# blacksnail789521/IMM-TSF

Hardware: AMD Instinct MI355X
Metric: forecast windows/sec (train fwd+bwd) on ragged 64-entity batch (higher is better)
Workload: dtype bf16

## Files before the change

imm-tsf_amd/csrc/gemm.hip:

```cpp
#include "gemm.hpp"
#include "rowops.hpp"
#include <atomic>
#include <mutex>
#include <shared_mutex>

namespace {

typedef short s16x4 __attribute__((ext_vector_type(4)));
typedef short s16x8 __attribute__((ext_vector_type(8)));

template <bool BF16> struct LdsElem { typedef float T; };
template <> struct LdsElem<true> { typedef bf16_t T; };

__device__ __forceinline__ float gelu_erf(float x) { return 0.5f * x * (1.f + erff(x * 0.70710678118654752f)); }
__device__ __forceinline__ float gelu_erf_grad(float z) {
    return 0.5f * (1.f + erff(z * 0.70710678118654752f)) + z * 0.3989422804014327f * expf(-0.5f * z * z);
}

template <bool BF16, bool TR, int ROWS, int BK> struct TileGeom {
    static constexpr bool kmajor = BF16 && TR;
    static constexpr int pad = BF16 ? 8 : 1;
    static constexpr int pitch = kmajor ? (ROWS + 8) : (BK + pad);
    static constexpr int elems = kmajor ? BK * pitch : ROWS * pitch;
};
// ... 593 lines not shown
    switch (layout) {
        case GEMM_NT: hipLaunchKernelGGL((gemm_kernel<BF16, false, false, BM, BN, BK, WM, WN, SPEC, BBF>), grid, block, 0, stream, g); break;
        case GEMM_NN: hipLaunchKernelGGL((gemm_kernel<BF16, false, true, BM, BN, BK, WM, WN, SPEC, BBF>), grid, block, 0, stream, g); break;
        case GEMM_TN:
            if (BBF) return IMMTSF_EINVAL;
            hipLaunchKernelGGL((gemm_kernel<BF16, true, true, BM, BN, BK, WM, WN, SPEC, false>), grid, block, 0, stream, g);
            break;
        default: return IMMTSF_EINVAL;
    }
    IMMTSF_LAUNCH_CHECK();
    return IMMTSF_OK;
}

static int g_force_old = 0;

int g_variant = 0, g_splitk = 0, g_xcd = 1, g_dbg = 0, g_tn_spec = 1, g_xcd2d = 0;

}

void immtsf_gemm_note_grid(long threads) { g_last_grid_threads = threads; }

extern int g_immtsf_ttcn_fused;
extern int g_immtsf_ttcn_bwd_grid;

extern "C" int immtsf_debug_gemm_config(int variant, int splitk) {
    g_immtsf_ttcn_fused = (variant & 0x8000) ? 0 : 1;
    g_variant = variant & 0xff;
    g_xcd = (variant & 0x100) ? 0 : 1;
    g_dbg = (variant >> 9) & 15;
    g_tn_spec = (variant & 0x2000) ? 0 : 1;
    g_xcd2d = (variant & 0x4000) ? 1 : 0;
    g_force_old = (variant & 0x10000) ? 1 : 0;
    g_immtsf_ttcn_bwd_grid = (variant >> 17) & 1023;
    g_splitk = splitk;
    return 0;
}

namespace {
struct TapRec { hipEvent_t e0, e1; int meta[10]; int members[24]; };
constexpr int kTapCap = 16384;
TapRec* g_tap = nullptr;
int g_tap_n = 0, g_tap_events = 0;
std::atomic<int> g_tap_on{0};
std::mutex g_tap_mu;
}

static int launch_gemm_impl(int layout, int precision, GemmArgs& g, hipStream_t stream);

namespace {
struct TwinRange { const float* base; const unsigned short* twin; size_t count; };
constexpr int kMaxTwins = 16;
TwinRange g_twins[kMaxTwins];
int g_ntwins = 0;
std::atomic<int> g_twins_on{1};
std::shared_mutex g_twins_mu;
}
// ... 375 lines not shown
```

imm-tsf_amd/csrc/ttcn.hip:

```cpp
#include "ttcn.hpp"
#include "../../include/immtsf.h"
#include "block_util.hpp"
#include "rowops.hpp"

int g_immtsf_ttcn_fused = 1;

namespace {

constexpr int LC = 32;

struct Dims { int P, L, F, K, NC, Fp, Kp, NCp, R; };
inline int r4(int x) { return (x + 31) / 32 * 32; }
inline Dims mk_dims(int P, int L, int te_dim, int K) {
    Dims d;
    d.P = P; d.L = L; d.F = 1 + te_dim; d.K = K; d.NC = d.F * K;
    d.Fp = r4(d.F); d.Kp = r4(K); d.NCp = r4(d.NC); d.R = P * L;
    return d;
}

__global__ __launch_bounds__(256) void build_x_kernel(Dims d, const float* __restrict__ x, const float* __restrict__ tt,
                                                       const float* ws, const float* bs, const float* __restrict__ wp,
                                                       const float* __restrict__ bp, float* __restrict__ X) {
    const long idx = (long)blockIdx.x * 256 + threadIdx.x;
    if (idx >= (long)d.R * d.Fp) return;
// ... 91 lines not shown
    const float* mp = mask + (size_t)p * d.L;
    for (int l0 = 0; l0 < d.L; l0 += LC) {
        const int lcnt = min(LC, d.L - l0);
        if (col) {
            for (int l = 0; l < lcnt; ++l) {
                const float smd = Sp[(size_t)(l0 + l) * d.NCp] * dpk;
                smt[l * d.NC + c] = smd;
                Sp[(size_t)(l0 + l) * d.NCp] = smd * (Xp[(size_t)(l0 + l) * d.Fp + fc] - ct) * mp[l0 + l];
            }
        }
        __syncthreads();
        for (int i = c; i < lcnt * d.Fp; i += nt) {
            const int l = i / d.Fp, f = i % d.Fp;
            float a = 0.f;
            if (f < d.F) for (int k = 0; k < d.K; ++k) a += smt[l * d.NC + k * d.F + f];
            dX[((size_t)p * d.L + l0 + l) * d.Fp + f] = a;
        }
        __syncthreads();
    }
}

struct Ws {
    float *X, *h1, *h2, *S, *ctr, *W1p, *b1p, *W2p, *b2p, *W3p, *b3p, *pack;
    size_t bytes;
};
Ws carve_ws(const Dims& d, void* base) {
    Carver k(base);
    Ws w;
    w.X = k.take<float>((size_t)d.R * d.Fp);
    w.h1 = k.take<float>((size_t)d.R * d.Kp);
    w.h2 = k.take<float>((size_t)d.R * d.Kp);
    w.S = k.take<float>((size_t)d.R * d.NCp);
    w.ctr = k.take<float>((size_t)d.P * (d.NC > d.F * 32 ? d.NC : d.F * 32));
    w.W1p = k.take<float>(d.Kp * d.Fp);
    w.b1p = k.take<float>(d.Kp);
    w.W2p = k.take<float>(d.Kp * d.Kp);
    w.b2p = k.take<float>(d.Kp);
    w.W3p = k.take<float>((size_t)d.NCp * d.Kp);
    w.b3p = k.take<float>(d.NCp);
    w.pack = k.take<float>(ttcn_full_pack_floats(d.F));
    w.bytes = k.bytes();
    return w;
}
struct Sc {
    float *dX, *dpool, *dz2, *dz1, *gW1p, *gb1p, *gW2p, *gb2p, *gW3p, *gb3p, *red, *slab;
    size_t bytes;
};
Sc carve_sc(const Dims& d, void* base) {
    Carver k(base);
    Sc s;
    s.dX = k.take<float>((size_t)d.R * d.Fp);
    s.dpool = k.take<float>((size_t)d.P * d.K);
    s.dz2 = k.take<float>((size_t)d.R * d.Kp);
    s.dz1 = k.take<float>((size_t)d.R * d.Kp);
    s.gW1p = k.take<float>(d.Kp * d.Fp);
    s.gb1p = k.take<float>(d.Kp);
    s.gW2p = k.take<float>(d.Kp * d.Kp);
    s.gb2p = k.take<float>(d.Kp);
    s.gW3p = k.take<float>((size_t)d.NCp * d.Kp);
    s.gb3p = k.take<float>(d.NCp);
    s.red = k.take<float>(64 * (d.NCp + 64) + 2 * 256 * d.F);
    s.slab = k.take<float>(ttcn_full_slab_floats(d.F));
    s.bytes = k.bytes();
// ... 33 lines not shown
int immtsf_patch_flatten3(const float* x, const float* tt, const float* mask, int32_t B, int32_t M, int32_t L, int32_t N, float* ox,
                          float* ott, float* omask, immtsf_stream_t stream) {
    if (!x || !tt || !mask || !ox || !ott || !omask || B < 0 || M <= 0 || L <= 0 || N <= 0) return IMMTSF_EINVAL;
    const size_t total = (size_t)B * M * L * N;
    if (total == 0) return IMMTSF_OK;
    hipLaunchKernelGGL(patch_flatten3_kernel, dim3((unsigned)((total + 255) / 256)), dim3(256), 0, static_cast<hipStream_t>(stream), x, tt, mask,
                       B, M, L, N, ox, ott, omask);
    IMMTSF_LAUNCH_CHECK();
    return IMMTSF_OK;
}

int immtsf_ttcn_forward(int32_t P, int32_t L, int32_t te_dim, int32_t ttcn_dim, int32_t precision, const float* x,
                        const float* tt, const float* mask, const immtsf_ttcn_params* p, float* out, int32_t out_ld,
                        int32_t flag_col, void* workspace, size_t workspace_bytes, immtsf_stream_t stream) {
    if (!x || !tt || !mask || !p || !out || !workspace) return IMMTSF_EINVAL;
    if (out_ld < ttcn_dim || flag_col >= out_ld || (flag_col >= 0 && flag_col < ttcn_dim)) return IMMTSF_EINVAL;
    if (bad_dims(P, L, te_dim, ttcn_dim)) return (1 + te_dim) * ttcn_dim > 1024 ? IMMTSF_EUNSUPPORTED : IMMTSF_EINVAL;
    if (P == 0) return IMMTSF_OK;
    const Dims d = mk_dims(P, L, te_dim, ttcn_dim);
    Ws w = carve_ws(d, workspace);
    if (workspace_bytes < w.bytes) return IMMTSF_EWORKSPACE;
    hipStream_t s = static_cast<hipStream_t>(stream);
    if (g_immtsf_ttcn_fused && ttcn_full_supported(precision, L, d.F, d.K))
        return launch_ttcn_full_fwd(P, L, d.F, d.K, x, tt, mask, p, w.pack, w.ctr, out, out_ld, flag_col, s);
    PackPtrs q{p->W1, p->b1, p->W2, p->b2, p->W3, p->b3, w.W1p, w.b1p, w.W2p, w.b2p, w.W3p, w.b3p};
    hipLaunchKernelGGL(pack_w_kernel, dim3(cdiv(d.NCp * d.Kp, 256)), dim3(256), 0, s, d, q);
    IMMTSF_LAUNCH_CHECK();
    const long nx = (long)d.R * d.Fp;
    hipLaunchKernelGGL(build_x_kernel, dim3((unsigned)((nx + 255) / 256)), dim3(256), 0, s, d, x, tt, p->te_scale_w, p->te_scale_b,
                       p->te_per_w, p->te_per_b, w.X);
    IMMTSF_LAUNCH_CHECK();
    {
        GemmArgs g = gemm_args(d.R, d.Kp, d.Fp, d.Fp, d.Fp, d.Kp);
        set_problem(g, 0, w.X, w.W1p, w.h1, w.b1p);
        g.act = 1;
        CHECK(immtsf_launch_gemm(GEMM_NT, precision, g, s));
    }
    {
        GemmArgs g = gemm_args(d.R, d.Kp, d.Kp, d.Kp, d.Kp, d.Kp);
        set_problem(g, 0, w.h1, w.W2p, w.h2, w.b2p);
        g.act = 1;
        CHECK(immtsf_launch_gemm(GEMM_NT, precision, g, s));
    }
    {
        GemmArgs g = gemm_args(d.R, d.NCp, d.Kp, d.Kp, d.Kp, d.NCp);
        set_problem(g, 0, w.h2, w.W3p, w.S, w.b3p);
        CHECK(immtsf_launch_gemm(GEMM_NT, precision, g, s));
    }
    const int threads = cdiv(d.NC, 64) * 64;
    hipLaunchKernelGGL(pool_fwd_kernel, dim3(P), dim3(threads), d.NC * sizeof(float), s, d, w.S, w.X, mask, p->T_bias, w.ctr, out, out_ld, flag_col);
    IMMTSF_LAUNCH_CHECK();
    return IMMTSF_OK;
}

int immtsf_ttcn_backward(int32_t P, int32_t L, int32_t te_dim, int32_t ttcn_dim, int32_t precision, const float* x,
                         const float* tt, const float* mask, const immtsf_ttcn_params* p, const float* out,
                         const float* dout, int32_t out_ld, void* workspace, size_t workspace_bytes, void* scratch,
                         size_t scratch_bytes, const immtsf_ttcn_params* gr, int32_t te_accumulate, immtsf_stream_t stream) {
    if (!tt || !mask || !p || !out || !dout || !gr || !workspace || !scratch || out_ld < ttcn_dim) return IMMTSF_EINVAL;
    if (bad_dims(P, L, te_dim, ttcn_dim)) return IMMTSF_EINVAL;
    if (P == 0) return IMMTSF_OK;
    const Dims d = mk_dims(P, L, te_dim, ttcn_dim);
    Ws w = carve_ws(d, workspace);
    Sc sc = carve_sc(d, scratch);
    if (workspace_bytes < w.bytes || scratch_bytes < sc.bytes) return IMMTSF_EWORKSPACE;
    hipStream_t s = static_cast<hipStream_t>(stream);
    if (g_immtsf_ttcn_fused && ttcn_full_supported(precision, L, d.F, d.K))
        return launch_ttcn_full_bwd(P, L, d.F, d.K, x, tt, mask, p, w.pack, w.ctr, out, dout, out_ld, sc.slab, gr,
                                    static_cast<hipStream_t>(stream), te_accumulate);
    {
        const size_t nbytes = (size_t)((char*)(sc.gb3p + d.NCp) - (char*)sc.gW1p);
        if (int rc = launch_fill(sc.gW1p, 0.f, nbytes / sizeof(float), s)) return rc;
    }
    Fork fk(s);
    {
        const int threads = cdiv(d.NC, 64) * 64;
        const size_t lds = (size_t)(d.K + LC * d.NC) * sizeof(float);
        if (lds > 160 * 1024) return IMMTSF_EUNSUPPORTED;
        hipLaunchKernelGGL(pool_bwd_kernel, dim3(P), dim3(threads), lds, s, d, w.S, w.X, mask, w.ctr, out, dout, out_ld, sc.dX, sc.dpool);
        IMMTSF_LAUNCH_CHECK();
    }
    CHECK(launch_colsum(sc.dpool, nullptr, P, nullptr, d.K, d.K, gr->T_bias, 0, sc.red, s));
    {
        GemmArgs h = gemm_args(d.NCp, d.Kp, d.R, d.NCp, d.Kp, d.Kp);
        set_problem(h, 0, w.S, w.h2, sc.gW3p, nullptr, sc.gb3p);
        h.c_prezeroed = 1;
        CHECK(immtsf_launch_gemm(GEMM_TN, precision, h, fk.fork()));
        GemmArgs g = gemm_args(d.R, d.Kp, d.NCp, d.NCp, d.Kp, d.Kp);
        set_problem(g, 0, w.S, w.W3p, sc.dz2, nullptr);
        g.relu_ref = w.h2; g.ld_ref = d.Kp;
        CHECK(immtsf_launch_gemm(GEMM_NN, precision, g, s));
// ... 31 lines not shown
```

imm-tsf_amd/csrc/ttcn.hpp:

```cpp
#pragma once
#include "common.hpp"

struct immtsf_ttcn_params;
bool ttcn_full_supported(int precision, int L, int F, int K);
size_t ttcn_full_pack_floats(int F);
size_t ttcn_full_slab_floats(int F);
int launch_ttcn_full_fwd(int P, int L, int F, int K, const float* x, const float* tt, const float* mask, const immtsf_ttcn_params* p,
                         float* pack, float* ctr, float* out, int out_ld, int flag_col, hipStream_t s);
int launch_ttcn_full_bwd(int P, int L, int F, int K, const float* x, const float* tt, const float* mask, const immtsf_ttcn_params* p,
                         const float* pack, const float* ctr, const float* out, const float* dout, int out_ld, float* slab,
                         const immtsf_ttcn_params* gr, hipStream_t s, int te_acc = 0);
```

imm-tsf_amd/csrc/ttcn_full.hip:

```cpp
#include "ttcn.hpp"
#include "../../include/immtsf.h"
#include "common.hpp"
#include <stdio.h>
#include <stdlib.h>

int g_immtsf_ttcn_bwd_grid = 0;

namespace {

typedef short s16x8 __attribute__((ext_vector_type(8)));
typedef float f32x2 __attribute__((ext_vector_type(2)));

constexpr int KP = 32;
constexpr int PT = 40;


struct FD { int P, L, F, K, NCq, dbg; };

struct Slab { int W1, b1, W2, b2, W3, b3, te, Tb, total; };
__host__ __device__ inline Slab slab_of(int F) {
    Slab s;
    int o = 0;
    s.W1 = o; o += KP * KP;
    s.b1 = o; o += KP;
    s.W2 = o; o += KP * KP;
    s.b2 = o; o += KP;
    s.W3 = o; o += F * 32 * KP;
    s.b3 = o; o += F * 32;
    s.te = o; o += 2 * KP;
    s.Tb = o; o += KP;
    s.total = o;
    return s;
}

__device__ __forceinline__ bf16x8 load8_bf16(const float* __restrict__ src) {
    const float4 a = *reinterpret_cast<const float4*>(src), b = *reinterpret_cast<const float4*>(src + 4);
    bf16x8 r;
// ... 102 lines not shown
        const f32x4 acc = mfma(frag_row(in, PT, rt * 16, 0, fr, fq), load8_bf16(W + (nt * 16 + fr) * KP + fq * 8), zero4());
        const float bias = b[nt * 16 + fr];
#pragma unroll
        for (int r = 0; r < 4; ++r) outp[(rt * 16 + fq * 4 + r) * PT + nt * 16 + fr] = (bf16_t)fmaxf(acc[r] + bias, 0.f);
    }
}

template <int RT>
__device__ __forceinline__ void mlp_layer_frag(const bf16_t* in, bf16_t* outp, const bf16x8 wf, const float bias, int wave, int fr, int fq) {
    for (int t = wave; t < RT * 2; t += 4) {
        const int rt = t >> 1, nt = t & 1;
        const f32x4 acc = mfma(frag_row(in, PT, rt * 16, 0, fr, fq), wf, zero4());
#pragma unroll
        for (int r = 0; r < 4; ++r) outp[(rt * 16 + fq * 4 + r) * PT + nt * 16 + fr] = (bf16_t)fmaxf(acc[r] + bias, 0.f);
    }
}

struct Wts { const float *W1p, *b1p, *W2p, *b2p, *W3q, *b3q; };

template <int RT, int MF>
__global__ __launch_bounds__(256) void ttcn_full_fwd_kernel(FD d, const float* __restrict__ x, const float* __restrict__ tt,
                                                             const float* __restrict__ mask, TEp te, Wts w, const bf16_t* __restrict__ W3h,
                                                             const float* __restrict__ Tb, float* __restrict__ ctr,
                                                             float* __restrict__ out, int out_ld, int flag_col) {
    extern __shared__ __attribute__((aligned(16))) unsigned char smem[];
    constexpr int ROWS = RT * 16, XP = xt_pitch<RT>();
    constexpr float LOG2E = 1.4426950408889634f;
    bf16_t* Xb = reinterpret_cast<bf16_t*>(smem);
    bf16_t* h1s = Xb + ROWS * PT;
    bf16_t* h2s = h1s + ROWS * PT;
    float* Xf = reinterpret_cast<float*>(h2s + ROWS * PT);
    float* cl = Xf + 16 * XP;
    float* pin = cl + d.NCq;
    const int tid = threadIdx.x, lane = tid & 63, wave = tid >> 6, fr = lane & 15, fq = lane >> 4;
    bf16x8 bw[MF][2];
    float b3v[MF][2];
    const int tnt = wave & 1;
    typedef PatchIn<RT, false> PI;
    PI nx;
    nx.fetch(d, blockIdx.x, x, tt, mask, nullptr, nullptr, nullptr, 0);
    const XCol xc = x_col(d, te);
    const bf16x8 mw1 = load8_bf16(w.W1p + (tnt * 16 + fr) * KP + fq * 8), mw2 = load8_bf16(w.W2p + (tnt * 16 + fr) * KP + fq * 8);
    const float mb1 = w.b1p[tnt * 16 + fr], mb2 = w.b2p[tnt * 16 + fr];
    const float tb = tid < d.K ? Tb[tid] : 0.f;
#pragma unroll
    for (int j = 0; j < MF; ++j)
#pragma unroll
        for (int half = 0; half < 2; ++half) {
            const int f = wave + 4 * j, c = f * 32 + half * 16 + fr;
            bw[j][half] = bf16x8{0, 0, 0, 0, 0, 0, 0, 0};
            b3v[j][half] = 0.f;
            if (f < d.F) { bw[j][half] = *reinterpret_cast<const bf16x8*>(W3h + (size_t)c * KP + fq * 8); b3v[j][half] = w.b3q[c] * LOG2E; }
        }
    nx.park(d, pin);
    __syncthreads();
    int it = 0;
    for (int p = blockIdx.x; p < d.P; p += gridDim.x, ++it) {
    const float* cur = pin + (it & 1) * PI::HEAD;
    const int pn = p + gridDim.x;
    if (pn < d.P) nx.fetch(d, pn, x, tt, mask, nullptr, nullptr, nullptr, 0);
    build_x<RT, true>(d, xc, cur, Xb, Xf);
    __syncthreads();
    mlp_layer_frag<RT>(Xb, h1s, mw1, mb1, wave, fr, fq);
    __syncthreads();
    mlp_layer_frag<RT>(h1s, h2s, mw2, mb2, wave, fr, fq);
    __syncthreads();
    bf16x8 a[RT];
    bool on[RT][4];
    float cval[RT][4];
#pragma unroll
    for (int rt = 0; rt < RT; ++rt) {
        a[rt] = frag_row(h2s, PT, rt * 16, 0, fr, fq);
        const f32x4 m4 = *reinterpret_cast<const f32x4*>(cur + 2 * ROWS + rt * 16 + fq * 4);
#pragma unroll
        for (int r = 0; r < 4; ++r) {
            on[rt][r] = m4[r] != 0.f;
            cval[rt][r] = rt * 16 + fq * 4 + r < d.L ? -1e8f * LOG2E : -INFINITY;
        }
    }
#pragma unroll
    for (int j = 0; j < MF; ++j) {
        const int f = wave + 4 * j;
        if (f < d.F) {
// ... 23 lines not shown
                            m = fmaxf(m, v[rt][h][e]);
                        }
                }
                m = col_max(m);
                f32x2 s2{0.f, 0.f}, p2{0.f, 0.f};
#pragma unroll
                for (int rt = 0; rt < RT; ++rt)
#pragma unroll
                    for (int h = 0; h < 2; ++h) {
                        v[rt][h] -= m;
                        v[rt][h][0] = __builtin_amdgcn_exp2f(v[rt][h][0]);
                        v[rt][h][1] = __builtin_amdgcn_exp2f(v[rt][h][1]);
                        s2 += v[rt][h];
                        p2 += v[rt][h] * xf[rt][h];
                    }
                const float acc = col_sum(p2[0] + p2[1]) * __builtin_amdgcn_rcpf(col_sum(s2[0] + s2[1]));
                if (fq == 0) {
                    cl[c] = acc;
                    ctr[(size_t)p * d.NCq + c] = acc;
                }
            }
        }
    }
    if (pn < d.P) nx.park(d, pin + ((it + 1) & 1) * PI::HEAD);
    __syncthreads();
    if (tid < d.K) {
        float s = tb;
        for (int f = 0; f < d.F; ++f) s += cl[f * 32 + tid];
        out[(size_t)p * out_ld + tid] = fmaxf(s, 0.f);
    }
    if (flag_col >= 0 && wave == 1) {
        float any = lane < d.L ? cur[2 * ROWS + lane] : 0.f;
        any = wave_sum(any);
        if (lane == 0) out[(size_t)p * out_ld + flag_col] = any > 0.f ? 1.f : 0.f;
    }
    __syncthreads();
    }
}

struct WtsT { const bf16_t *W3T , *W2T , *W1T , *W3h ; };

template <int RT, int MF>
__global__ __launch_bounds__(256) __attribute__((amdgpu_waves_per_eu(RT == 2 ? 2 : 1))) void ttcn_full_bwd_kernel(FD d, const float* __restrict__ x, const float* __restrict__ tt,
                                                             const float* __restrict__ mask, TEp te, Wts w, WtsT wt,
                                                             const float* __restrict__ ctr, const float* __restrict__ out,
                                                             const float* __restrict__ dout, int out_ld, float* __restrict__ slab) {
    extern __shared__ __attribute__((aligned(16))) unsigned char smem[];
    constexpr int ROWS = RT * 16, PTT = ROWS + 8, XP = xt_pitch<RT>();
    constexpr float LOG2E = 1.4426950408889634f;
    bf16_t* Xb = reinterpret_cast<bf16_t*>(smem);
    bf16_t* h1s = Xb + ROWS * PT;
    bf16_t* h2s = h1s + ROWS * PT;
    bf16_t* dz2s = h2s + ROWS * PT;
    bf16_t* dz1s = h2s;
    bf16_t* dST = dz2s + ROWS * PT;
    float* Xf = reinterpret_cast<float*>(dST + d.NCq * PTT);
    float* Xc = Xf + 16 * XP;
    typedef PatchIn<RT, true> PI;
    const int PIN = PI::HEAD + d.NCq;
    float* pin = Xc + 16 * XP;
    bf16_t* W3s = reinterpret_cast<bf16_t*>(pin + 2 * PIN);
    bf16_t* W1s = W3s + d.NCq * PT;
    bf16_t* W2s = W1s + KP * PT;
    float* b3s = reinterpret_cast<float*>(W2s + KP * PT);
    const int tid = threadIdx.x, lane = tid & 63, wave = tid >> 6, fr = lane & 15, fq = lane >> 4;
    const Slab sl = slab_of(d.F);
    PI nx;
    nx.fetch(d, blockIdx.x, x, tt, mask, ctr, out, dout, out_ld);
    const XCol xc = x_col(d, te);
    for (int i = tid; i < d.NCq * 4; i += 256) {
        const int c = i >> 2, q = i & 3;
        *reinterpret_cast<bf16x8*>(W3s + c * PT + q * 8) = *reinterpret_cast<const bf16x8*>(wt.W3h + (size_t)c * KP + q * 8);
    }
    for (int i = tid; i < d.NCq; i += 256) b3s[i] = w.b3q[i] * LOG2E;
    if (tid < 2 * KP * 4) {
        const int which = tid >> 7, r = (tid >> 2) & 31, q = tid & 3;
        *reinterpret_cast<bf16x8*>((which ? W2s : W1s) + r * PT + q * 8) = load8_bf16((which ? w.W2p : w.W1p) + r * KP + q * 8);
    }

    f32x4 accW3[MF][2][2];
    f32x2 accB3[MF][2];
#pragma unroll
    for (int j = 0; j < MF; ++j)
#pragma unroll
        for (int half = 0; half < 2; ++half) {
            accW3[j][half][0] = zero4(); accW3[j][half][1] = zero4();
            accB3[j][half] = f32x2{0.f, 0.f};
        }
    const int tnt = wave & 1, tmt = wave >> 1;
    const float mb1 = w.b1p[tnt * 16 + fr], mb2 = w.b2p[tnt * 16 + fr];
    f32x4 accW2 = zero4(), accW1 = zero4();
    float sb2 = 0.f, sb1 = 0.f;
    float accT = 0.f;
    float te_w = 0.f, te_b = 0.f;
    f32x2 tpw[MF], tpb[MF];
#pragma unroll
    for (int j = 0; j < MF; ++j) tpw[j] = tpb[j] = f32x2{0.f, 0.f};

    nx.park(d, pin);
    __syncthreads();
    int it = 0;
    for (int p = blockIdx.x; p < d.P; p += gridDim.x, ++it) {
        const float* cur = pin + (it & 1) * PIN;
        const float *dp = cur + 3 * ROWS, *cts = cur + PI::HEAD;
        const int pn = p + gridDim.x;
        if (pn < d.P) nx.fetch(d, pn, x, tt, mask, ctr, out, dout, out_ld);
        build_x<RT, true>(d, xc, cur, Xb, Xf, Xc);
        __syncthreads();
        if (tid >= 128 && tid < 128 + KP) accT += dp[tid - 128];
        mlp_layer_frag<RT>(Xb, h1s, frag_row(W1s, PT, tnt * 16, 0, fr, fq), mb1, wave, fr, fq);
        __syncthreads();
        mlp_layer_frag<RT>(h1s, h2s, frag_row(W2s, PT, tnt * 16, 0, fr, fq), mb2, wave, fr, fq);
        __syncthreads();
        bf16x8 a[RT];
        bool on[RT][4];
        float cval[RT][4], anyf = 0.f;
        f32x4 t4[RT];
#pragma unroll
        for (int rt = 0; rt < RT; ++rt) {
            a[rt] = frag_row(h2s, PT, rt * 16, 0, fr, fq);
            t4[rt] = *reinterpret_cast<const f32x4*>(cur + rt * 16 + fq * 4);
            const f32x4 m4 = *reinterpret_cast<const f32x4*>(cur + 2 * ROWS + rt * 16 + fq * 4);
#pragma unroll
            for (int r = 0; r < 4; ++r) {
                on[rt][r] = m4[r] != 0.f;
                cval[rt][r] = rt * 16 + fq * 4 + r < d.L ? -1e8f * LOG2E : -INFINITY;
                anyf += on[rt][r] ? 1.f : 0.f;
            }
        }
// ... 108 lines not shown
                const int o = (rt * 16 + fq * 4 + r) * PT + tnt * 16 + fr;
                const float g = (float)h1s[o] > 0.f ? acc[r] : 0.f;
                dz1s[o] = (bf16_t)g;
                sb1 += g;
            }
        }
        __syncthreads();
        if (wave < 2) {
#pragma unroll
            for (int kk = 0; kk < ROWS; kk += 32)
                accW1 = mfma(frag_kmajor(dz1s, PT, wave * 16, kk, fr, fq), frag_kmajor(Xb, PT, 0, kk, fr, fq), accW1);
        }
        for (int rt = (RT == 2 ? wave - 2 : wave); rt >= 0 && rt < RT; rt += 4) {
            const f32x4 acc = mfma(frag_row(dz1s, PT, rt * 16, 0, fr, fq), frag_kmajor(W1s, PT, 0, 0, fr, fq), zero4());
            const f32x4 c4 = *reinterpret_cast<const f32x4*>(Xc + fr * XP + rt * 16 + fq * 4);
            const f32x4 tr = *reinterpret_cast<const f32x4*>(cur + rt * 16 + fq * 4);
#pragma unroll
            for (int r = 0; r < 4; ++r) {
                const float g = acc[r] * c4[r];
                te_w = fmaf(g, tr[r], te_w);
                te_b += g;
            }
        }
        if (pn < d.P) nx.park(d, pin + ((it + 1) & 1) * PIN);
        __syncthreads();
    }

    float* my = slab + (size_t)blockIdx.x * sl.total;
#pragma unroll
    for (int j = 0; j < MF; ++j) {
        const int f = wave + 4 * j;
        if (f < d.F) {
#pragma unroll
            for (int half = 0; half < 2; ++half) {
#pragma unroll
                for (int nt = 0; nt < 2; ++nt)
#pragma unroll
                    for (int r = 0; r < 4; ++r)
                        my[sl.W3 + (size_t)(f * 32 + half * 16 + fq * 4 + r) * KP + nt * 16 + fr] = accW3[j][half][nt][r];
                const float b3sum = col_sum(accB3[j][half][0] + accB3[j][half][1]);
                if (fq == 0) my[sl.b3 + f * 32 + half * 16 + fr] = b3sum;
            }
        }
    }
#pragma unroll
    for (int r = 0; r < 4; ++r) {
        my[sl.W2 + (tmt * 16 + fq * 4 + r) * KP + tnt * 16 + fr] = accW2[r];
        if (wave < 2) my[sl.W1 + (wave * 16 + fq * 4 + r) * KP + fr] = accW1[r];
    }
    if (tid >= 128 && tid < 128 + KP) my[sl.Tb + tid - 128] = accT;
    float* tes = pin;
    if (tid < 4 * KP) tes[tid] = 0.f;
    __syncthreads();
#pragma unroll
    for (int j = 0; j < MF; ++j) {
        const int f = wave + 4 * j;
        const float sw = col_sum(row_sum16(tpw[j][0] + tpw[j][1])), sb = col_sum(row_sum16(tpb[j][0] + tpb[j][1]));
        if (lane == 0 && f >= 1 && f < d.F) {
            atomicAdd(tes + f, sw);
            atomicAdd(tes + KP + f, sb);
        }
    }
    te_w = col_sum(te_w);
    te_b = col_sum(te_b);
    sb2 = col_sum(sb2);
    sb1 = col_sum(sb1);
    if (fq == 0) {
        if (RT == 4 || wave >= 2) {
            atomicAdd(tes + fr, te_w);
            atomicAdd(tes + KP + fr, te_b);
        }
        atomicAdd(tes + 2 * KP + tnt * 16 + fr, sb2);
        atomicAdd(tes + 3 * KP + tnt * 16 + fr, sb1);
    }
    __syncthreads();
    if (tid < 2 * KP) my[sl.te + tid] = tes[tid];
    else if (tid < 3 * KP) my[sl.b2 + tid - 2 * KP] = tes[tid];
    else if (tid < 4 * KP) my[sl.b1 + tid - 3 * KP] = tes[tid];
}

struct PackIn { const float *W1, *b1, *W2, *b2, *W3, *b3; };
__global__ __launch_bounds__(256) void ttcn_pack_kernel(int F, int K, PackIn q, float* W1p, float* b1p, float* W2p, float* b2p,
                                                         float* W3q, float* b3q, bf16_t* W3T, bf16_t* W2T, bf16_t* W1T, bf16_t* W3h) {
    const int i = blockIdx.x * 256 + threadIdx.x, NCq = F * 32;
    if (i < KP * KP) {
        const int r = i >> 5, c = i & 31;
        const float v1 = (r < K && c < F) ? q.W1[r * F + c] : 0.f, v2 = (r < K && c < K) ? q.W2[r * K + c] : 0.f;
        W1p[i] = v1;
        W2p[i] = v2;
        W1T[c * KP + r] = (bf16_t)v1;
        W2T[c * KP + r] = (bf16_t)v2;
    }
    if (i < KP) { b1p[i] = i < K ? q.b1[i] : 0.f; b2p[i] = i < K ? q.b2[i] : 0.f; }
    if (i < NCq * KP) {
        const int c = i >> 5, kk = i & 31, f = c >> 5, k = c & 31;
        const float v = (k < K && kk < K) ? q.W3[(size_t)(k * F + f) * K + kk] : 0.f;
        W3q[i] = v;
        W3T[(size_t)kk * NCq + c] = (bf16_t)v;
        W3h[i] = (bf16_t)v;
    }
    if (i < NCq) { const int f = i >> 5, k = i & 31; b3q[i] = k < K ? q.b3[k * F + f] : 0.f; }
}

struct UnpackOut { float *W1, *b1, *W2, *b2, *W3, *b3, *ws, *bs, *wp, *bp, *Tb; };
__global__ __launch_bounds__(256) void ttcn_unpack_kernel(int F, int K, const float* __restrict__ slab, int nslab, UnpackOut g, int te_acc) {
    __shared__ float red[8][33];
    const Slab sl = slab_of(F);
    const int slot = threadIdx.x & 31, part = threadIdx.x >> 5;
    int i = blockIdx.x * 32 + slot, n;
    float* dst = nullptr;
    int off = 0;
    bool acc = false;
    if (i < (n = K * F)) { dst = g.W1 + i; off = sl.W1 + (i / F) * KP + i % F; }
    else if ((i -= n) < (n = K * K)) { dst = g.W2 + i; off = sl.W2 + (i / K) * KP + i % K; }
    else if ((i -= n) < (n = F * K * K)) { const int c = i / K, kk = i % K, k = c / F, f = c % F; dst = g.W3 + i; off = sl.W3 + (f * 32 + k) * KP + kk; }
    else if ((i -= n) < (n = F * K)) { const int k = i / F, f = i % F; dst = g.b3 + i; off = sl.b3 + f * 32 + k; }
    else if ((i -= n) < K) { dst = g.b1 + i; off = sl.b1 + i; }
    else if ((i -= K) < K) { dst = g.b2 + i; off = sl.b2 + i; }
    else if ((i -= K) < K) { dst = g.Tb + i; off = sl.Tb + i; }
    else if ((i -= K) < 1) { dst = g.ws; off = sl.te + 1; acc = te_acc != 0; }
    else if ((i -= 1) < 1) { dst = g.bs; off = sl.te + KP + 1; acc = te_acc != 0; }
    else if ((i -= 1) < F - 2) { dst = g.wp + i; off = sl.te + 2 + i; acc = te_acc != 0; }
    else if ((i -= F - 2) < F - 2) { dst = g.bp + i; off = sl.te + KP + 2 + i; acc = te_acc != 0; }
    float s = 0.f;
    if (dst) {
#pragma unroll 8
        for (int w = part; w < nslab; w += 8) s += slab[(size_t)w * sl.total + off];
    }
    red[part][slot] = s;
    __syncthreads();
    if (part == 0 && dst) {
#pragma unroll
        for (int q = 1; q < 8; ++q) s += red[q][slot];
        *dst = (acc ? *dst : 0.f) + s;
    }
}
inline int ttcn_unpack_outputs(int F, int K) { return K * F + K * K + F * K * K + F * K + 3 * K + 2 + 2 * (F - 2); }
constexpr int kMaxBwdGrid = 512;

size_t fwd_lds(int RT, int NCq) { return (size_t)RT * 16 * PT * 2 * 3 + (size_t)16 * (RT * 16 + 4) * 4 + (size_t)NCq * 4 + (size_t)2 * 3 * RT * 16 * 4 + 64; }
size_t bwd_lds(int RT, int NCq) {
    const size_t ROWS = RT * 16;
    return ROWS * PT * 2 * 4 + (size_t)NCq * (ROWS + 8) * 2 + 16 * (ROWS + 4) * 4 * 2 + 2 * (3 * ROWS + KP + (size_t)NCq) * 4 + (size_t)(NCq + 2 * KP) * PT * 2 + (size_t)NCq * 4;
}

struct PackPtrs { float *W1p, *b1p, *W2p, *b2p, *W3q, *b3q; bf16_t *W3T, *W2T, *W1T, *W3h; };
PackPtrs pack_ptrs(float* base, int F) {
    PackPtrs q;
    float* o = base;
    q.W1p = o; o += KP * KP;
    q.W2p = o; o += KP * KP;
    q.b1p = o; o += KP;
    q.b2p = o; o += KP;
    q.W3q = o; o += (size_t)F * 32 * KP;
    q.b3q = o; o += F * 32;
    q.W3T = reinterpret_cast<bf16_t*>(o); o += (size_t)F * 32 * KP / 2;
    q.W2T = reinterpret_cast<bf16_t*>(o); o += KP * KP / 2;
    q.W1T = reinterpret_cast<bf16_t*>(o); o += KP * KP / 2;
    q.W3h = reinterpret_cast<bf16_t*>(o);
    return q;
}

}

bool ttcn_full_supported(int precision, int L, int F, int K) {
    return precision == 1 && K >= 1 && K <= 32 && F >= 2 && F <= 16 && L >= 1 && L <= 64;
}
size_t ttcn_full_pack_floats(int F) { return (size_t)2 * KP * KP + 2 * KP + (size_t)F * 32 * KP + F * 32 + (size_t)F * 32 * KP + KP * KP + 64; }
size_t ttcn_full_slab_floats(int F) { return (size_t)kMaxBwdGrid * slab_of(F).total; }

int launch_ttcn_full_fwd(int P, int L, int F, int K, const float* x, const float* tt, const float* mask, const immtsf_ttcn_params* p,
                         float* pack, float* ctr, float* out, int out_ld, int flag_col, hipStream_t s) {
    const FD d{P, L, F, K, F * 32};
    const PackPtrs q = pack_ptrs(pack, F);
    hipLaunchKernelGGL(ttcn_pack_kernel, dim3(cdiv(F * 32 * KP, 256)), dim3(256), 0, s, F, K, PackIn{p->W1, p->b1, p->W2, p->b2, p->W3, p->b3},
                       q.W1p, q.b1p, q.W2p, q.b2p, q.W3q, q.b3q, q.W3T, q.W2T, q.W1T, q.W3h);
    IMMTSF_LAUNCH_CHECK();
    const TEp te{p->te_scale_w, p->te_scale_b, p->te_per_w, p->te_per_b};
    const Wts w{q.W1p, q.b1p, q.W2p, q.b2p, q.W3q, q.b3q};
    const int mf = (F + 3) / 4;
#define TTCN_FWD(RT, MF)                                                                                                                     \
    hipLaunchKernelGGL((ttcn_full_fwd_kernel<RT, MF>), dim3(P < 2048 ? P : 2048), dim3(256), fwd_lds(RT, d.NCq), s, d, x, tt, mask, te, w, q.W3h, p->T_bias, ctr, \
                       out, out_ld, flag_col)
    if (L <= 32) {
        if (mf == 1) TTCN_FWD(2, 1); else if (mf == 2) TTCN_FWD(2, 2); else if (mf == 3) TTCN_FWD(2, 3); else TTCN_FWD(2, 4);
    } else {
        if (mf == 1) TTCN_FWD(4, 1); else if (mf == 2) TTCN_FWD(4, 2); else if (mf == 3) TTCN_FWD(4, 3); else TTCN_FWD(4, 4);
    }
#undef TTCN_FWD
    IMMTSF_LAUNCH_CHECK();
    return IMMTSF_OK;
}

int launch_ttcn_full_bwd(int P, int L, int F, int K, const float* x, const float* tt, const float* mask, const immtsf_ttcn_params* p,
                         const float* pack, const float* ctr, const float* out, const float* dout, int out_ld, float* slab,
                         const immtsf_ttcn_params* gr, hipStream_t s, int te_acc) {
    const FD d{P, L, F, K, F * 32, 0};
    const PackPtrs q = pack_ptrs(const_cast<float*>(pack), F);
    const TEp te{p->te_scale_w, p->te_scale_b, p->te_per_w, p->te_per_b};
    const Wts w{q.W1p, q.b1p, q.W2p, q.b2p, q.W3q, q.b3q};
    const WtsT wt{q.W3T, q.W2T, q.W1T, q.W3h};
    const int genv = g_immtsf_ttcn_bwd_grid;
    int gmax = genv > 0 ? genv : (L <= 32 ? (P >= 8192 ? 512 : 384) : 224);
    gmax = gmax > kMaxBwdGrid ? kMaxBwdGrid : gmax;
    const int grid = P < gmax ? P : gmax;
    const size_t lds = bwd_lds(L <= 32 ? 2 : 4, d.NCq);
    const int mf = (F + 3) / 4;
#define TTCN_BWD(RT, MF)                                                                                                                  \
    do {                                                                                                                                  \
        if (lds > 64 * 1024)                                                                                                              \
            (void)hipFuncSetAttribute(reinterpret_cast<const void*>(ttcn_full_bwd_kernel<RT, MF>), hipFuncAttributeMaxDynamicSharedMemorySize, \
                                      (int)lds);                                                                                          \
        hipLaunchKernelGGL((ttcn_full_bwd_kernel<RT, MF>), dim3(grid), dim3(256), lds, s, d, x, tt, mask, te, w, wt, ctr, out, dout, out_ld, \
                           slab);                                                                                                         \
    } while (0)
    if (L <= 32) {
        if (mf == 1) TTCN_BWD(2, 1); else if (mf == 2) TTCN_BWD(2, 2); else if (mf == 3) TTCN_BWD(2, 3); else TTCN_BWD(2, 4);
    } else {
        if (mf == 1) TTCN_BWD(4, 1); else if (mf == 2) TTCN_BWD(4, 2); else if (mf == 3) TTCN_BWD(4, 3); else TTCN_BWD(4, 4);
    }
#undef TTCN_BWD
    IMMTSF_LAUNCH_CHECK();
    hipLaunchKernelGGL(ttcn_unpack_kernel, dim3(cdiv(ttcn_unpack_outputs(F, K), 32)), dim3(256), 0, s, F, K, slab, grid,
                       UnpackOut{gr->W1, gr->b1, gr->W2, gr->b2, gr->W3, gr->b3, gr->te_scale_w, gr->te_scale_b, gr->te_per_w, gr->te_per_b,
                                 gr->T_bias}, te_acc);
    IMMTSF_LAUNCH_CHECK();
    return IMMTSF_OK;
}
```

Before: 156,700.

## Skip MLP for fully-masked TTCN patches and rebalance backward work lists

The forward kernel detects patches whose mask is entirely zero, records a per-patch live flag, and takes a short path that computes only the masked-mean centre instead of running the full MLP. The backward kernel builds per-block work lists from those flags, spreading live and dead patches evenly across blocks. Dead patches get a cheap gradient path that touches only the time-embedding and T_bias terms. Blocks left without work can exit early, and the unpack kernel reads how many slabs were actually written. This targets the wasted work on ragged batches with many empty patches, at the cost of extra LDS, a prefix scan, and more code complexity.

```diff
diff --git a/imm-tsf_amd/csrc/gemm.hip b/imm-tsf_amd/csrc/gemm.hip
--- a/imm-tsf_amd/csrc/gemm.hip
+++ b/imm-tsf_amd/csrc/gemm.hip
@@ -639,6 +639,7 @@
 
 extern int g_immtsf_ttcn_fused;
 extern int g_immtsf_ttcn_bwd_grid;
+extern int g_immtsf_ttcn_live;
 
 extern "C" int immtsf_debug_gemm_config(int variant, int splitk) {
     g_immtsf_ttcn_fused = (variant & 0x8000) ? 0 : 1;
@@ -649,6 +650,7 @@
     g_xcd2d = (variant & 0x4000) ? 1 : 0;
     g_force_old = (variant & 0x10000) ? 1 : 0;
     g_immtsf_ttcn_bwd_grid = (variant >> 17) & 1023;
+    g_immtsf_ttcn_live = 7 & ~(variant >> 27);
     g_splitk = splitk;
     return 0;
 }
diff --git a/imm-tsf_amd/csrc/ttcn.hip b/imm-tsf_amd/csrc/ttcn.hip
--- a/imm-tsf_amd/csrc/ttcn.hip
+++ b/imm-tsf_amd/csrc/ttcn.hip
@@ -137,6 +137,7 @@
 
 struct Ws {
     float *X, *h1, *h2, *S, *ctr, *W1p, *b1p, *W2p, *b2p, *W3p, *b3p, *pack;
+    unsigned char* live;
     size_t bytes;
 };
 Ws carve_ws(const Dims& d, void* base) {
@@ -154,6 +155,7 @@
     w.W3p = k.take<float>((size_t)d.NCp * d.Kp);
     w.b3p = k.take<float>(d.NCp);
     w.pack = k.take<float>(ttcn_full_pack_floats(d.F));
+    w.live = k.take<unsigned char>(ttcn_full_live_bytes());
     w.bytes = k.bytes();
     return w;
 }
@@ -233,7 +235,7 @@
     if (workspace_bytes < w.bytes) return IMMTSF_EWORKSPACE;
     hipStream_t s = static_cast<hipStream_t>(stream);
     if (g_immtsf_ttcn_fused && ttcn_full_supported(precision, L, d.F, d.K))
-        return launch_ttcn_full_fwd(P, L, d.F, d.K, x, tt, mask, p, w.pack, w.ctr, out, out_ld, flag_col, s);
+        return launch_ttcn_full_fwd(P, L, d.F, d.K, x, tt, mask, p, w.pack, w.ctr, w.live, out, out_ld, flag_col, s);
     PackPtrs q{p->W1, p->b1, p->W2, p->b2, p->W3, p->b3, w.W1p, w.b1p, w.W2p, w.b2p, w.W3p, w.b3p};
     hipLaunchKernelGGL(pack_w_kernel, dim3(cdiv(d.NCp * d.Kp, 256)), dim3(256), 0, s, d, q);
     IMMTSF_LAUNCH_CHECK();
@@ -277,7 +279,7 @@
     if (workspace_bytes < w.bytes || scratch_bytes < sc.bytes) return IMMTSF_EWORKSPACE;
     hipStream_t s = static_cast<hipStream_t>(stream);
     if (g_immtsf_ttcn_fused && ttcn_full_supported(precision, L, d.F, d.K))
-        return launch_ttcn_full_bwd(P, L, d.F, d.K, x, tt, mask, p, w.pack, w.ctr, out, dout, out_ld, sc.slab, gr,
+        return launch_ttcn_full_bwd(P, L, d.F, d.K, x, tt, mask, p, w.pack, w.ctr, w.live, out, dout, out_ld, sc.slab, gr,
                                     static_cast<hipStream_t>(stream), te_accumulate);
     {
         const size_t nbytes = (size_t)((char*)(sc.gb3p + d.NCp) - (char*)sc.gW1p);
diff --git a/imm-tsf_amd/csrc/ttcn.hpp b/imm-tsf_amd/csrc/ttcn.hpp
--- a/imm-tsf_amd/csrc/ttcn.hpp
+++ b/imm-tsf_amd/csrc/ttcn.hpp
@@ -5,8 +5,9 @@
 bool ttcn_full_supported(int precision, int L, int F, int K);
 size_t ttcn_full_pack_floats(int F);
 size_t ttcn_full_slab_floats(int F);
+size_t ttcn_full_live_bytes();
 int launch_ttcn_full_fwd(int P, int L, int F, int K, const float* x, const float* tt, const float* mask, const immtsf_ttcn_params* p,
-                         float* pack, float* ctr, float* out, int out_ld, int flag_col, hipStream_t s);
+                         float* pack, float* ctr, unsigned char* live, float* out, int out_ld, int flag_col, hipStream_t s);
 int launch_ttcn_full_bwd(int P, int L, int F, int K, const float* x, const float* tt, const float* mask, const immtsf_ttcn_params* p,
-                         const float* pack, const float* ctr, const float* out, const float* dout, int out_ld, float* slab,
-                         const immtsf_ttcn_params* gr, hipStream_t s, int te_acc = 0);
+                         const float* pack, const float* ctr, const unsigned char* live, const float* out, const float* dout, int out_ld,
+                         float* slab, const immtsf_ttcn_params* gr, hipStream_t s, int te_acc = 0);
diff --git a/imm-tsf_amd/csrc/ttcn_full.hip b/imm-tsf_amd/csrc/ttcn_full.hip
--- a/imm-tsf_amd/csrc/ttcn_full.hip
+++ b/imm-tsf_amd/csrc/ttcn_full.hip
@@ -5,6 +5,7 @@
 #include <stdlib.h>
 
 int g_immtsf_ttcn_bwd_grid = 0;
+int g_immtsf_ttcn_live = 7;
 
 namespace {
 
@@ -13,6 +14,8 @@
 
 constexpr int KP = 32;
 constexpr int PT = 40;
+constexpr int kMaxList = 64;
+constexpr int kLiveMaxP = 8192;
 
 
 struct FD { int P, L, F, K, NCq, dbg; };
@@ -161,7 +164,8 @@
 __global__ __launch_bounds__(256) void ttcn_full_fwd_kernel(FD d, const float* __restrict__ x, const float* __restrict__ tt,
                                                              const float* __restrict__ mask, TEp te, Wts w, const bf16_t* __restrict__ W3h,
                                                              const float* __restrict__ Tb, float* __restrict__ ctr,
-                                                             float* __restrict__ out, int out_ld, int flag_col) {
+                                                             float* __restrict__ out, int out_ld, int flag_col,
+                                                             unsigned char* __restrict__ live, int short_path) {
     extern __shared__ __attribute__((aligned(16))) unsigned char smem[];
     constexpr int ROWS = RT * 16, XP = xt_pitch<RT>();
     constexpr float LOG2E = 1.4426950408889634f;
@@ -198,6 +202,42 @@
     const float* cur = pin + (it & 1) * PI::HEAD;
     const int pn = p + gridDim.x;
     if (pn < d.P) nx.fetch(d, pn, x, tt, mask, nullptr, nullptr, nullptr, 0);
+    const bool empty = live != nullptr && __ballot(lane < d.L && cur[2 * ROWS + lane] != 0.f) == 0;
+    if (live != nullptr && tid == 0) live[p] = empty ? 0 : 1;
+    if (empty && short_path) {
+        const float invL = __builtin_amdgcn_rcpf((float)d.L);
+#pragma unroll
+        for (int j = 0; j < MF; ++j) {
+            const int f = wave + 4 * j;
+            if (f < d.F) {
+                const float tw = f == 0 ? 0.f : f == 1 ? te.ws[0] : te.wp[f - 2], tbs = f == 0 ? 0.f : f == 1 ? te.bs[0] : te.bp[f - 2];
+                f32x2 p2{0.f, 0.f};
+#pragma unroll
+                for (int rt = 0; rt < RT; ++rt) {
+                    const f32x4 t4 = *reinterpret_cast<const f32x4*>(cur + rt * 16 + fq * 4);
+                    const f32x4 x4 = *reinterpret_cast<const f32x4*>(cur + ROWS + rt * 16 + fq * 4);
+                    float xv[4];
+#pragma unroll
+                    for (int r = 0; r < 4; ++r) {
+                        const float ph = fmaf(tw, t4[r], tbs);
+                        const float v = f == 0 ? x4[r] : f == 1 ? ph : __sinf(ph);
+                        xv[r] = rt * 16 + fq * 4 + r < d.L ? v : 0.f;
+                    }
+                    p2 += f32x2{xv[0], xv[1]};
+                    p2 += f32x2{xv[2], xv[3]};
+                }
+                const float acc = col_sum(p2[0] + p2[1]) * invL;
+                if (fq == 0) {
+#pragma unroll
+                    for (int half = 0; half < 2; ++half) {
+                        const int c = f * 32 + half * 16 + fr;
+                        cl[c] = acc;
+                        ctr[(size_t)p * d.NCq + c] = acc;
+                    }
+                }
+            }
+        }
+    } else {
     build_x<RT, true>(d, xc, cur, Xb, Xf);
     __syncthreads();
     mlp_layer_frag<RT>(Xb, h1s, mw1, mb1, wave, fr, fq);
@@ -267,6 +307,7 @@
             }
         }
     }
+    }
     if (pn < d.P) nx.park(d, pin + ((it + 1) & 1) * PI::HEAD);
     __syncthreads();
     if (tid < d.K) {
@@ -289,7 +330,8 @@
 __global__ __launch_bounds__(256) __attribute__((amdgpu_waves_per_eu(RT == 2 ? 2 : 1))) void ttcn_full_bwd_kernel(FD d, const float* __restrict__ x, const float* __restrict__ tt,
                                                              const float* __restrict__ mask, TEp te, Wts w, WtsT wt,
                                                              const float* __restrict__ ctr, const float* __restrict__ out,
-                                                             const float* __restrict__ dout, int out_ld, float* __restrict__ slab) {
+                                                             const float* __restrict__ dout, int out_ld, float* __restrict__ slab,
+                                                             const unsigned char* __restrict__ live, int* __restrict__ nslab) {
     extern __shared__ __attribute__((aligned(16))) unsigned char smem[];
     constexpr int ROWS = RT * 16, PTT = ROWS + 8, XP = xt_pitch<RT>();
     constexpr float LOG2E = 1.4426950408889634f;
@@ -310,9 +352,75 @@
     float* b3s = reinterpret_cast<float*>(W2s + KP * PT);
     const int tid = threadIdx.x, lane = tid & 63, wave = tid >> 6, fr = lane & 15, fq = lane >> 4;
     const Slab sl = slab_of(d.F);
+    float* tep = b3s + d.NCq;
+    int* wtot = reinterpret_cast<int*>(tep + 32);
+    unsigned short* list = reinterpret_cast<unsigned short*>(wtot + 8);
+
+    int nmine;
+    if (live != nullptr) {
+        unsigned word = 0;
+        const int p0 = tid * 32;
+        if (p0 < d.P) {
+            const uint4 a = reinterpret_cast<const uint4*>(live)[tid * 2], b = reinterpret_cast<const uint4*>(live)[tid * 2 + 1];
+            const unsigned u[8] = {a.x, a.y, a.z, a.w, b.x, b.y, b.z, b.w};
+#pragma unroll
+            for (int q = 0; q < 8; ++q) word |= ((u[q] & 1u) | ((u[q] >> 7) & 2u) | ((u[q] >> 14) & 4u) | ((u[q] >> 21) & 8u)) << (4 * q);
+            if (d.P - p0 < 32) word &= (1u << (d.P - p0)) - 1u;
+        }
+        const int cnt = __popc(word);
+        int inc = cnt;
+#pragma unroll
+        for (int o = 1; o < 64; o <<= 1) {
+            const int v = __shfl_up(inc, o);
+            if (lane >= o) inc += v;
+        }
+        if (lane == 63) wtot[wave] = inc;
+        __syncthreads();
+        int base = inc - cnt, nlive = 0;
+#pragma unroll
+        for (int q = 0; q < 4; ++q) {
+            const int t = wtot[q];
+            if (q < wave) base += t;
+            nlive += t;
+        }
+        const int ndead = d.P - nlive, G = gridDim.x, b = blockIdx.x;
+        const int rounds = nlive > G ? (nlive + G - 1) / G : 1;
+        int ge = max((nlive + rounds - 1) / rounds, (ndead + 3) / 4);
+        ge = max(min(ge, G), 1);
+        if (b >= ge) {
+            if (nslab == nullptr)
+                for (int i = tid; i < sl.total; i += 256) slab[(size_t)b * sl.total + i] = 0.f;
+            return;
+        }
+        if (nslab != nullptr && b == 0 && tid == 0) *nslab = ge;
+        const int bd = ge - 1 - b;
+        const int nl = nlive > b ? (nlive - b - 1) / ge + 1 : 0, nd = ndead > bd ? (ndead - bd - 1) / ge + 1 : 0;
+        nmine = min(nl + nd, kMaxList);
+        if (p0 < d.P) {
+            int rl = base % ge, ql = base / ge, rd = (p0 - base) % ge, qd = (p0 - base) / ge;
+            const int n = min(32, d.P - p0);
+            for (int i = 0; i < n; ++i) {
+                if ((word >> i) & 1u) {
+                    if (rl == b && ql < kMaxList) list[ql] = (unsigned short)(p0 + i);
+                    if (++rl == ge) { rl = 0; ++ql; }
+                } else {
+                    if (rd == bd && nl + qd < kMaxList) list[nl + qd] = (unsigned short)((p0 + i) | 0x8000);
+                    if (++rd == ge) { rd = 0; ++qd; }
+                }
+            }
+        }
+        __syncthreads();
+    } else {
+        nmine = (d.P - (int)blockIdx.x + (int)gridDim.x - 1) / (int)gridDim.x;
+    }
+    auto patch_of = [&](int i) -> int { return live != nullptr ? (list[i] & 0x7fff) : (int)(blockIdx.x + i * gridDim.x); };
     PI nx;
-    nx.fetch(d, blockIdx.x, x, tt, mask, ctr, out, dout, out_ld);
+    nx.fetch(d, patch_of(0), x, tt, mask, ctr, out, dout, out_ld);
     const XCol xc = x_col(d, te);
+    if (tid < 32) {
+        const int f = tid & 15, which = tid >> 4;
+        tep[tid] = f == 1 ? (which ? te.bs[0] : te.ws[0]) : (f >= 2 && f < d.F) ? (which ? te.bp[f - 2] : te.wp[f - 2]) : 0.f;
+    }
     for (int i = tid; i < d.NCq * 4; i += 256) {
         const int c = i >> 2, q = i & 3;
         *reinterpret_cast<bf16x8*>(W3s + c * PT + q * 8) = *reinterpret_cast<const bf16x8*>(wt.W3h + (size_t)c * KP + q * 8);
@@ -344,12 +452,39 @@
 
     nx.park(d, pin);
     __syncthreads();
-    int it = 0;
-    for (int p = blockIdx.x; p < d.P; p += gridDim.x, ++it) {
+    for (int it = 0; it < nmine; ++it) {
         const float* cur = pin + (it & 1) * PIN;
         const float *dp = cur + 3 * ROWS, *cts = cur + PI::HEAD;
-        const int pn = p + gridDim.x;
-        if (pn < d.P) nx.fetch(d, pn, x, tt, mask, ctr, out, dout, out_ld);
+        const bool more = it + 1 < nmine;
+        if (more) nx.fetch(d, patch_of(it + 1), x, tt, mask, ctr, out, dout, out_ld);
+        if (live != nullptr && (list[it] & 0x8000)) {
+            if (tid >= 128 && tid < 128 + KP) accT += dp[tid - 128];
+            const float invL = __builtin_amdgcn_rcpf((float)d.L);
+            const float dsum = dp[fr] * invL + dp[16 + fr] * invL;
+#pragma unroll
+            for (int j = 0; j < MF; ++j) {
+                const int f = wave + 4 * j;
+                if (f >= 1 && f < d.F) {
+                    const float tw = tep[f], tbs = tep[16 + f];
+#pragma unroll
+                    for (int rt = 0; rt < RT; ++rt) {
+                        const f32x4 t4 = *reinterpret_cast<const f32x4*>(cur + rt * 16 + fq * 4);
+                        float g[4];
+#pragma unroll
+                        for (int r = 0; r < 4; ++r) {
+                            const float c = f == 1 ? 1.f : __cosf(fmaf(tw, t4[r], tbs));
+                            g[r] = rt * 16 + fq * 4 + r < d.L ? dsum * c : 0.f;
+                        }
+                        const f32x2 g0{g[0], g[1]}, g1{g[2], g[3]};
+                        tpb[j] += g0 + g1;
+                        tpw[j] += g0 * f32x2{t4[0], t4[1]} + g1 * f32x2{t4[2], t4[3]};
+                    }
+                }
+            }
+            if (more) nx.park(d, pin + ((it + 1) & 1) * PIN);
+            __syncthreads();
+            continue;
+        }
         build_x<RT, true>(d, xc, cur, Xb, Xf, Xc);
         __syncthreads();
         if (tid >= 128 && tid < 128 + KP) accT += dp[tid - 128];
@@ -504,7 +639,7 @@
                 te_b += g;
             }
         }
-        if (pn < d.P) nx.park(d, pin + ((it + 1) & 1) * PIN);
+        if (more) nx.park(d, pin + ((it + 1) & 1) * PIN);
         __syncthreads();
     }
 
@@ -547,16 +682,22 @@
     te_b = col_sum(te_b);
     sb2 = col_sum(sb2);
     sb1 = col_sum(sb1);
+    float* tem = tes + 4 * KP;
     if (fq == 0) {
         if (RT == 4 || wave >= 2) {
-            atomicAdd(tes + fr, te_w);
-            atomicAdd(tes + KP + fr, te_b);
+            tem[wave * 2 * KP + fr] = te_w;
+            tem[wave * 2 * KP + KP + fr] = te_b;
         }
         atomicAdd(tes + 2 * KP + tnt * 16 + fr, sb2);
         atomicAdd(tes + 3 * KP + tnt * 16 + fr, sb1);
     }
     __syncthreads();
-    if (tid < 2 * KP) my[sl.te + tid] = tes[tid];
+    if (tid < 2 * KP) {
+        float v = tes[tid];
+        if ((tid & 31) < 16)
+            for (int q = RT == 4 ? 0 : 2; q < 4; ++q) v += tem[q * 2 * KP + tid];
+        my[sl.te + tid] = v;
+    }
     else if (tid < 3 * KP) my[sl.b2 + tid - 2 * KP] = tes[tid];
     else if (tid < 4 * KP) my[sl.b1 + tid - 3 * KP] = tes[tid];
 }
@@ -585,9 +726,11 @@
 }
 
 struct UnpackOut { float *W1, *b1, *W2, *b2, *W3, *b3, *ws, *bs, *wp, *bp, *Tb; };
-__global__ __launch_bounds__(256) void ttcn_unpack_kernel(int F, int K, const float* __restrict__ slab, int nslab, UnpackOut g, int te_acc) {
+__global__ __launch_bounds__(256) void ttcn_unpack_kernel(int F, int K, const float* __restrict__ slab, int nslab, const int* __restrict__ written,
+                                                           UnpackOut g, int te_acc) {
     __shared__ float red[8][33];
     const Slab sl = slab_of(F);
+    if (written != nullptr) nslab = min(nslab, *written);
     const int slot = threadIdx.x & 31, part = threadIdx.x >> 5;
     int i = blockIdx.x * 32 + slot, n;
     float* dst = nullptr;
@@ -623,7 +766,8 @@
 size_t fwd_lds(int RT, int NCq) { return (size_t)RT * 16 * PT * 2 * 3 + (size_t)16 * (RT * 16 + 4) * 4 + (size_t)NCq * 4 + (size_t)2 * 3 * RT * 16 * 4 + 64; }
 size_t bwd_lds(int RT, int NCq) {
     const size_t ROWS = RT * 16;
-    return ROWS * PT * 2 * 4 + (size_t)NCq * (ROWS + 8) * 2 + 16 * (ROWS + 4) * 4 * 2 + 2 * (3 * ROWS + KP + (size_t)NCq) * 4 + (size_t)(NCq + 2 * KP) * PT * 2 + (size_t)NCq * 4;
+    return ROWS * PT * 2 * 4 + (size_t)NCq * (ROWS + 8) * 2 + 16 * (ROWS + 4) * 4 * 2 + 2 * (3 * ROWS + KP + (size_t)NCq) * 4 + (size_t)(NCq + 2 * KP) * PT * 2 + (size_t)NCq * 4 +
+           (32 + 8) * 4 + kMaxList * 2;
 }
 
 struct PackPtrs { float *W1p, *b1p, *W2p, *b2p, *W3q, *b3q; bf16_t *W3T, *W2T, *W1T, *W3h; };
@@ -649,10 +793,11 @@
     return precision == 1 && K >= 1 && K <= 32 && F >= 2 && F <= 16 && L >= 1 && L <= 64;
 }
 size_t ttcn_full_pack_floats(int F) { return (size_t)2 * KP * KP + 2 * KP + (size_t)F * 32 * KP + F * 32 + (size_t)F * 32 * KP + KP * KP + 64; }
-size_t ttcn_full_slab_floats(int F) { return (size_t)kMaxBwdGrid * slab_of(F).total; }
+size_t ttcn_full_slab_floats(int F) { return (size_t)kMaxBwdGrid * slab_of(F).total + 64; }
+size_t ttcn_full_live_bytes() { return kLiveMaxP; }
 
 int launch_ttcn_full_fwd(int P, int L, int F, int K, const float* x, const float* tt, const float* mask, const immtsf_ttcn_params* p,
-                         float* pack, float* ctr, float* out, int out_ld, int flag_col, hipStream_t s) {
+                         float* pack, float* ctr, unsigned char* live, float* out, int out_ld, int flag_col, hipStream_t s) {
     const FD d{P, L, F, K, F * 32};
     const PackPtrs q = pack_ptrs(pack, F);
     hipLaunchKernelGGL(ttcn_pack_kernel, dim3(cdiv(F * 32 * KP, 256)), dim3(256), 0, s, F, K, PackIn{p->W1, p->b1, p->W2, p->b2, p->W3, p->b3},
@@ -661,9 +806,11 @@
     const TEp te{p->te_scale_w, p->te_scale_b, p->te_per_w, p->te_per_b};
     const Wts w{q.W1p, q.b1p, q.W2p, q.b2p, q.W3q, q.b3q};
     const int mf = (F + 3) / 4;
+    unsigned char* lv = P < kLiveMaxP ? live : nullptr;
+    const int sp = (g_immtsf_ttcn_live & 2) ? 1 : 0;
 #define TTCN_FWD(RT, MF)                                                                                                                     \
     hipLaunchKernelGGL((ttcn_full_fwd_kernel<RT, MF>), dim3(P < 2048 ? P : 2048), dim3(256), fwd_lds(RT, d.NCq), s, d, x, tt, mask, te, w, q.W3h, p->T_bias, ctr, \
-                       out, out_ld, flag_col)
+                       out, out_ld, flag_col, lv, sp)
     if (L <= 32) {
         if (mf == 1) TTCN_FWD(2, 1); else if (mf == 2) TTCN_FWD(2, 2); else if (mf == 3) TTCN_FWD(2, 3); else TTCN_FWD(2, 4);
     } else {
@@ -675,8 +822,8 @@
 }
 
 int launch_ttcn_full_bwd(int P, int L, int F, int K, const float* x, const float* tt, const float* mask, const immtsf_ttcn_params* p,
-                         const float* pack, const float* ctr, const float* out, const float* dout, int out_ld, float* slab,
-                         const immtsf_ttcn_params* gr, hipStream_t s, int te_acc) {
+                         const float* pack, const float* ctr, const unsigned char* live, const float* out, const float* dout, int out_ld,
+                         float* slab, const immtsf_ttcn_params* gr, hipStream_t s, int te_acc) {
     const FD d{P, L, F, K, F * 32, 0};
     const PackPtrs q = pack_ptrs(const_cast<float*>(pack), F);
     const TEp te{p->te_scale_w, p->te_scale_b, p->te_per_w, p->te_per_b};
@@ -686,6 +833,9 @@
     int gmax = genv > 0 ? genv : (L <= 32 ? (P >= 8192 ? 512 : 384) : 224);
     gmax = gmax > kMaxBwdGrid ? kMaxBwdGrid : gmax;
     const int grid = P < gmax ? P : gmax;
+    const bool wl = (g_immtsf_ttcn_live & 1) && live != nullptr && P < kLiveMaxP && 2 * cdiv(P, grid) + 4 <= kMaxList;
+    const unsigned char* lv = wl ? live : nullptr;
+    int* nslab = wl && (g_immtsf_ttcn_live & 4) ? reinterpret_cast<int*>(slab + (size_t)kMaxBwdGrid * slab_of(F).total) : nullptr;
     const size_t lds = bwd_lds(L <= 32 ? 2 : 4, d.NCq);
     const int mf = (F + 3) / 4;
 #define TTCN_BWD(RT, MF)                                                                                                                  \
@@ -694,7 +844,7 @@
             (void)hipFuncSetAttribute(reinterpret_cast<const void*>(ttcn_full_bwd_kernel<RT, MF>), hipFuncAttributeMaxDynamicSharedMemorySize, \
                                       (int)lds);                                                                                          \
         hipLaunchKernelGGL((ttcn_full_bwd_kernel<RT, MF>), dim3(grid), dim3(256), lds, s, d, x, tt, mask, te, w, wt, ctr, out, dout, out_ld, \
-                           slab);                                                                                                         \
+                           slab, lv, nslab);                                                                                                        \
     } while (0)
     if (L <= 32) {
         if (mf == 1) TTCN_BWD(2, 1); else if (mf == 2) TTCN_BWD(2, 2); else if (mf == 3) TTCN_BWD(2, 3); else TTCN_BWD(2, 4);
@@ -704,7 +854,7 @@
 #undef TTCN_BWD
     IMMTSF_LAUNCH_CHECK();
     hipLaunchKernelGGL(ttcn_unpack_kernel, dim3(cdiv(ttcn_unpack_outputs(F, K), 32)), dim3(256), 0, s, F, K, slab, grid,
-                       UnpackOut{gr->W1, gr->b1, gr->W2, gr->b2, gr->W3, gr->b3, gr->te_scale_w, gr->te_scale_b, gr->te_per_w, gr->te_per_b,
+                       nslab, UnpackOut{gr->W1, gr->b1, gr->W2, gr->b2, gr->W3, gr->b3, gr->te_scale_w, gr->te_scale_b, gr->te_per_w, gr->te_per_b,
                                  gr->T_bias}, te_acc);
     IMMTSF_LAUNCH_CHECK();
     return IMMTSF_OK;
```

New measurement: 155,100. 1.0% lower.
